# lrmantovani10/Stable-Diffusion.mojo

Measured on AMD Instinct MI355X. Metric: UNet denoising steps/sec @ 512x512 latent, batch=8, higher is better.
Workload: dtype f16; 1 GPU; Tiny-SD UNet 512x512 (latent 4x64x64), batch 8/GPU, 50-step DDPM schedule, 77-token context, no CFG, random-init weights (BASELINE configs[1]); global_batch=8, parallelism=dp1 (independent prompts, weights broadcast once)

## Files before the change

include/tsd.h:

```cpp
#ifndef TSD_H
#define TSD_H

#include <stddef.h>
#include <stdint.h>

#ifdef __cplusplus
extern "C" {
#endif

#define TSD_VERSION 100

typedef enum tsd_status {
  TSD_OK = 0,
  TSD_E_ARG = -1,
  TSD_E_SHAPE = -2,
  TSD_E_ALLOC = -3,
  TSD_E_HIP = -4,
  TSD_E_RCCL = -5,
  TSD_E_STATE = -6,
  TSD_E_NONFINITE = -7
} tsd_status;

typedef struct tsd_ctx tsd_ctx;
typedef struct tsd_model tsd_model;
// ... 310 lines not shown
enum tsd_elem_mode {
  TSD_EM_SMALL_LINEAR = 0, TSD_EM_TIME_EMBEDDING, TSD_EM_GEGLU_ERF, TSD_EM_QUICK_GELU, TSD_EM_UNARY, TSD_EM_CLIP_EMBED,
  TSD_EM_CHW_TO_NHWC, TSD_EM_IM2COL3X3, TSD_EM_NHWC_TO_CHW, TSD_EM_F32_TO_F16_ROWS, TSD_EM_F16_TO_F32_ROWS, TSD_EM_TRANSPOSE_TO_F16,
  TSD_EM_PACK_CONV, TSD_EM_PACK_LINEAR, TSD_EM_PACK_BIAS, TSD_EM_PACK_IM2COL_W, TSD_EM_ENCODER_SAMPLE, TSD_EM_COUNT
};
enum tsd_elem_operand { TSD_EO_X = 0, TSD_EO_W, TSD_EO_BIAS, TSD_EO_Y, TSD_EO_COUNT };
enum tsd_elem_info { TSD_EI_CHANGED = 0, TSD_EI_NONFINITE, TSD_EI_NB, TSD_EI_PASSES, TSD_EI_COUNT };
int tsd_debug_elem_run(tsd_ctx* ctx, const int64_t* desc, int n, const void* const* host_in, void* const* host_out, int64_t* ext,
                       int64_t* info);
int tsd_debug_gn_path_counts(tsd_ctx* ctx, int64_t* counts, int n, int reset);
int tsd_debug_jitter_selftest(tsd_ctx* ctx, int n);
int tsd_debug_model_fold(tsd_model* m, int block, void* wf, float* bf);
int tsd_debug_model_dup_fold(tsd_model* m, void* conv1_w, void* skip_w);
int64_t tsd_debug_dup_fold_host(const void* w, int rows, int taps, int ldw, int half, void* out, int ldo);
int64_t tsd_debug_ups_fold_host(const void* w, int O, int Ipad, int ldw, void* out);
int tsd_debug_model_ups_fold(tsd_model* m, int block, void* out);
int tsd_debug_set_ups_fold(tsd_ctx* ctx, int on);
int tsd_debug_model_packed_param(tsd_model* m, int index, void* out, size_t cap);
int tsd_debug_attn_bench(tsd_ctx* ctx, int B, int H, int d, int Sq, int Sk, int iters, float* ms);
int tsd_debug_attn_exact_passes(tsd_ctx* ctx, int reset);
int tsd_debug_set_attn_qb(tsd_ctx* ctx, int mode);
int tsd_debug_set_attn_diag(tsd_ctx* ctx, int on);
int tsd_debug_set_res_fuse_skip(tsd_ctx* ctx, int on);
int tsd_debug_set_qkv_fuse(tsd_ctx* ctx, int on);
int tsd_debug_set_session_hoist(tsd_ctx* ctx, int on);
int tsd_debug_set_control_stats(tsd_ctx* ctx, int on);
int tsd_debug_session_hoist_info(tsd_session* s, int64_t* info);
int tsd_debug_mfma_sustained(tsd_ctx* ctx, float ms_target, float* tflops, float* clock_ghz);

double tsd_flop_count(int kind, int L, int T);

#ifdef __cplusplus
}
#endif
#endif
```

stable-diffusion.mojo_amd/csrc/common.h:

```cpp
#pragma once
#include <hip/hip_runtime.h>
#include <stdint.h>
#include <stdio.h>
#include <string>
#include <vector>

#include "../../include/tsd.h"
#include "counter_rng.h"

typedef _Float16 half_t;

void tsd_set_error(const char* fmt, ...);
#define TSD_FAIL(code, ...)      \
  do {                           \
    tsd_set_error(__VA_ARGS__);  \
    return (code);               \
  } while (0)
#define HIP_TRY(expr)                                                                              \
  do {                                                                                             \
    hipError_t e__ = (expr);                                                                       \
    if (e__ != hipSuccess) TSD_FAIL(TSD_E_HIP, "%s failed: %s (%s:%d)", #expr, hipGetErrorString(e__), __FILE__, __LINE__); \
  } while (0)
#define TSD_TRY(expr)            \
  do {                           \
// ... 3 lines not shown

struct Arena {
  char* base = nullptr;
  size_t cap = 0, top = 0, peak = 0;
  bool planning = false;
  size_t mark() const { return top; }
  void release(size_t m) { top = m; }
  void* alloc(size_t bytes) {
    size_t a = (top + 255) & ~size_t(255);
    size_t n = a + bytes;
    if (n > peak) peak = n;
    if (!planning && n > cap) return nullptr;
    top = n;
    return planning ? (void*)(uintptr_t)(0x1000 + a) : (void*)(base + a);
  }
};

struct TsdOptions {
  int qkv_fuse = 1;
  int res_fuse_skip = 1;
  int gn_composite = 1;
  int conv_in_im2col = 1;
  int chain = 1;
  int fold_out = 1;
  int ups_fold = 1;
  int fold_dup = 1;
  int control_stats = 1;
  int session_hoist = 1;
  int conv_w_tm_mib = 2, lin_w_tm = 1, lin_w_tm_kib = 1024;
  int attn_qb = 2;
  int attn_qb_force = 0;
  int attn_wg8 = 1;
  int attn8_var = 0;
  int attn_diag = 1;
  int attn_xcd = 0;
  int xcdn = 0, conv_halo = 0, splitk = 1, splitk_mink = 4096, splitk_tiles = 256, splitk_small = 8, splitk_wide = 1, splitk_ring4 = 0,
      splitk_big = 0, sk_cfg = 5, thin_cfg = 0, tune = 15, sk256 = 0, skip128 = 1;
  int force_cfg = -1;
  int sk_big_graph = 0;
  char cfg_override[512] = "";
  int gn_apply_mult = 2;
  int gn_finalize_min = 2048;
  int debug_occ = 0;
  int debug_poison_what = 7;
  int debug_poison = -1;
  int bench_wrot = 1, bench_epi = 0, bench_altcfg = -1, gemm_ts = 0;
// ... 386 lines not shown
  const half_t* Vt = nullptr; int ldvt = 0; int64_t sVt = 0;
  half_t* O = nullptr; int ldo = 0; int64_t sO = 0;
  const float* s = nullptr;
  int B = 0, H = 0, d = 0, S = 0, N = 0;
  float scale = 1.f;
};
int launch_ip_attn_add(tsd_ctx* ctx, const IpAttnArgs& a);

struct AttnTailArgs {
  const half_t* ao = nullptr; int ld_ao = 0;
  const half_t* tok = nullptr; int ld_tok = 0;
  const half_t* x = nullptr; int ld_x = 0;
  half_t* out = nullptr; int ld_out = 0;
  const half_t* wstream = nullptr;
  const float *bso = nullptr, *bco = nullptr, *b1 = nullptr, *b2 = nullptr, *bout = nullptr;
  const half_t* Kc = nullptr; int ldk = 0; int64_t sK = 0;
  const half_t* Vt = nullptr; int ldvt = 0; int64_t sVt = 0;
  int C = 0, d = 0, heads = 0, T = 0, S = 0; int64_t M = 0;
  float scale = 1.f, eps = 1e-5f;
  float* gn_part = nullptr; int gn_nslab = 0;
};
bool attn_tail_supported(const tsd_ctx* ctx, int C, int d, int heads, int T, int64_t M, int S);
int launch_attn_tail(tsd_ctx* ctx, const AttnTailArgs& a);
size_t attn_tail_stream_bytes();
struct AttnHeadArgs {
  const half_t* x = nullptr; int ld_x = 0;
  const float* gn_stats = nullptr;
  const half_t* wstream = nullptr;
  const float* b_in = nullptr;
  half_t* tok = nullptr; int ld_tok = 0;
  half_t* qk = nullptr; int ld_qk = 0;
  half_t* vt = nullptr; int ld_vt = 0; int64_t s_vt = 0;
  int64_t M = 0; int S = 0; float eps = 1e-5f;
};
size_t attn_head_stream_bytes();
int launch_attn_head_pack(tsd_ctx* ctx, const half_t* Wc, int ld_c, const half_t* Win, int ld_in, half_t* dst);
int launch_attn_head(tsd_ctx* ctx, const AttnHeadArgs& a);
int launch_gn_stats(tsd_ctx* ctx, const half_t* x, int ld, int B, int HW, int C, int groups, float eps, float gamma, float* stats);
int launch_gn_finalize(tsd_ctx* ctx, const float* partial, int nslab, int B, int HW, int C, int groups, float eps, float gamma,
                       float* stats);
int launch_attn_tail_pack(tsd_ctx* ctx, const half_t* Wso, int ld_so, const half_t* Wq, int ld_q, const half_t* Wco, int ld_co,
                          const half_t* W1, int ld_1, const half_t* W2, int ld_2, const half_t* Wout, int ld_out, half_t* dst);
int launch_flash_attention(tsd_ctx* ctx, const AttnArgs& a);

enum { CV_SIDE = 224, CV_PATCH = 14, CV_GRID = 16, CV_PATCHES = 256, CV_PATCH_K = 588, CV_PATCH_LD = 592 };
int vision_tab(tsd_ctx* ctx, int H, int W, VisionTab* out);
// ... 3 lines not shown
```

stable-diffusion.mojo_amd/csrc/kernels_chain.hip:

```cpp
#include <math.h>
#include <stdlib.h>

#include <atomic>
#include <type_traits>

#include "common.h"
#include "lds_dma.h"

#ifndef TSD_CHAIN_ABL
#define TSD_CHAIN_ABL 0
#endif
#ifndef TSD_CHAIN_TILE_BARRIER
#define TSD_CHAIN_TILE_BARRIER 0
#endif
#ifndef TSD_CHAIN_ARES
#define TSD_CHAIN_ARES 0
#endif

typedef _Float16 h8 __attribute__((ext_vector_type(8)));
typedef _Float16 h4 __attribute__((ext_vector_type(4)));
typedef _Float16 h2 __attribute__((ext_vector_type(2)));
typedef float f4 __attribute__((ext_vector_type(4)));
typedef float f2 __attribute__((ext_vector_type(2)));

// ... 865 lines not shown
int launch_attn_tail_pack(tsd_ctx* ctx, const half_t* Wso, int ld_so, const half_t* Wq, int ld_q, const half_t* Wco, int ld_co,
                          const half_t* W1, int ld_1, const half_t* W2, int ld_2, const half_t* Wout, int ld_out, half_t* dst) {
  if (ld_so < 320 || ld_q < 320 || ld_co < 320 || ld_1 < 320 || ld_2 < 1280 || ld_out < 320)
    TSD_FAIL(TSD_E_SHAPE, "attention tail: unexpected weight pitches");
  if (!ctx->launch()) return TSD_OK;
  const int n = STREAM_BYTES / 16;
  hipLaunchKernelGGL(k_attn_tail_pack, dim3(ceil_div(n, 256)), dim3(256), 0, ctx->stream, PackSrc{Wso, ld_so}, PackSrc{Wq, ld_q},
                     PackSrc{Wco, ld_co}, PackSrc{W1, ld_1}, PackSrc{W2, ld_2}, PackSrc{Wout, ld_out}, dst);
  HIP_TRY(hipGetLastError());
  return TSD_OK;
}

int launch_attn_tail(tsd_ctx* ctx, const AttnTailArgs& a) {
  if (!attn_tail_supported(ctx, a.C, a.d, a.heads, a.T, a.M, a.S)) TSD_FAIL(TSD_E_SHAPE, "attention tail: unsupported shape");
  if (!a.wstream) TSD_FAIL(TSD_E_ARG, "attention tail: weights were not packed");
  if (a.ld_ao % 8 || a.ld_tok % 8 || a.ld_x % 8 || a.ld_out % 8 || a.ldk % 8 || a.ldvt % 8 || a.ld_ao < 320 || a.ld_tok < 320 ||
      a.ld_x < 320 || a.ld_out < 320 || a.ldk < 320 || a.ldvt < ((a.T + 7) & ~7))
    TSD_FAIL(TSD_E_SHAPE, "attention tail: misaligned or too narrow pitches");
  if ((long long)a.M * a.ld_ao * 2 >= 0x7ffffff0LL) TSD_FAIL(TSD_E_SHAPE, "attention tail: ao operand exceeds the 2 GiB addressing window");
  if (!a.ao || !a.tok || !a.x || !a.out || !a.Kc || !a.Vt || !a.bso || !a.bco || !a.b1 || !a.b2 || !a.bout)
    TSD_FAIL(TSD_E_ARG, "attention tail: NULL operand");
  if (!ctx->launch()) return TSD_OK;
  ProfScope prof(ctx, KC_CHAIN, (int)a.M, a.C, 0, 1);
  TailK k;
  k.ao = a.ao; k.tok = a.tok; k.x = a.x; k.out = a.out;
  k.ld_ao = a.ld_ao; k.ld_tok = a.ld_tok; k.ld_x = a.ld_x; k.ld_out = a.ld_out;
  k.wstream = a.wstream;
  k.bso = a.bso; k.bco = a.bco; k.b1 = a.b1; k.b2 = a.b2; k.bout = a.bout;
  k.Kc = a.Kc; k.ldk = a.ldk; k.sK = a.sK; k.Vt = a.Vt; k.ldvt = a.ldvt; k.sVt = a.sVt;
  k.T = a.T; k.M = (int)a.M; k.S = a.S;
  k.qscale = a.scale * 1.4426950408889634f; k.eps = a.eps;
  k.gn_part = a.gn_part; k.gn_nslab = a.gn_nslab;
  k.gn_stats = nullptr; k.b_in = nullptr; k.tok_out = nullptr; k.qk = nullptr; k.ld_qk = 0; k.vt = nullptr; k.ld_vt = 0; k.s_vt = 0;
  static std::atomic<unsigned long long> attr{0};
  if (!((attr.load(std::memory_order_relaxed) >> (ctx->device & 63)) & 1)) {
    HIP_TRY(hipFuncSetAttribute((const void*)attn_chain_kernel<KIND_TAIL>, hipFuncAttributeMaxDynamicSharedMemorySize, LDS_BYTES));
    attr.fetch_or(1ull << (ctx->device & 63), std::memory_order_relaxed);
  }
  hipLaunchKernelGGL(attn_chain_kernel<KIND_TAIL>, dim3((unsigned)(a.M / BM)), dim3(256), LDS_BYTES, ctx->stream, k);
  HIP_TRY(hipGetLastError());
  return TSD_OK;
}

size_t attn_head_stream_bytes() { return (size_t)HEAD_STREAM_BYTES; }

int launch_attn_head_pack(tsd_ctx* ctx, const half_t* Wc, int ld_c, const half_t* Win, int ld_in, half_t* dst) {
// ... 31 lines not shown
```

stable-diffusion.mojo_amd/csrc/runtime.cpp:

```cpp
#include <stdarg.h>
#include <stdlib.h>
#include <string.h>

#include "common.h"

static thread_local char g_err[512] = "";

void tsd_set_error(const char* fmt, ...) {
  va_list ap;
  va_start(ap, fmt);
  vsnprintf(g_err, sizeof(g_err), fmt, ap);
  va_end(ap);
}

static int env_int(const char* name, int dflt) { const char* e = getenv(name); return e && *e ? atoi(e) : dflt; }
void options_from_env(TsdOptions& o) {
  o.qkv_fuse = env_int("TSD_QKV_FUSE", o.qkv_fuse);
  o.res_fuse_skip = env_int("TSD_RES_FUSE_SKIP", o.res_fuse_skip);
  o.gn_composite = env_int("TSD_GN_COMPOSITE", o.gn_composite);
  o.conv_in_im2col = env_int("TSD_CONV_IN_IM2COL", o.conv_in_im2col);
  o.chain = env_int("TSD_CHAIN", o.chain) ? 1 : 0;
  o.fold_out = env_int("TSD_FOLD_OUT", o.fold_out) ? 1 : 0;
  o.ups_fold = env_int("TSD_UPS_FOLD", o.ups_fold) ? 1 : 0;
  o.fold_dup = env_int("TSD_FOLD_DUP", o.fold_dup) ? 1 : 0;
  o.session_hoist = env_int("TSD_SESSION_HOIST", o.session_hoist) ? 1 : 0;
  o.control_stats = env_int("TSD_CONTROL_STATS", o.control_stats) ? 1 : 0;
  o.conv_w_tm_mib = env_int("TSD_CONV_W_TM", o.conv_w_tm_mib);
  o.lin_w_tm = env_int("TSD_LIN_W_TM", o.lin_w_tm);
  o.lin_w_tm_kib = env_int("TSD_LIN_W_TM_KIB", o.lin_w_tm_kib);
  { const int q = env_int("TSD_ATTN_QB", o.attn_qb); if (q == 1 || q == 2) o.attn_qb = q; }
  o.attn_xcd = env_int("TSD_ATTN_XCD", o.attn_xcd);
  o.attn_wg8 = env_int("TSD_ATTN_WG8", o.attn_wg8) ? 1 : 0;
  o.attn8_var = env_int("TSD_ATTN8_VAR", o.attn8_var);
  o.xcdn = env_int("TSD_GEMM_XCDN", o.xcdn);
  o.conv_halo = env_int("TSD_CONV_HALO", o.conv_halo);
  o.splitk = env_int("TSD_GEMM_SPLITK", o.splitk);
  o.splitk_mink = env_int("TSD_GEMM_SPLITK_MINK", o.splitk_mink);
  o.splitk_tiles = env_int("TSD_GEMM_SPLITK_TILES", o.splitk_tiles);
  o.splitk_small = env_int("TSD_GEMM_SPLITK_SMALL", o.splitk_small);
  o.splitk_wide = env_int("TSD_GEMM_SPLITK_WIDE", o.splitk_wide);
  o.splitk_ring4 = env_int("TSD_GEMM_SPLITK_RING4", o.splitk_ring4);
// ... 193 lines not shown
```

stable-diffusion.mojo_amd/tsd/_lib.py:

```python
import ctypes as C
import os

import numpy as np

_HERE = os.path.dirname(os.path.abspath(__file__))
LIB_PATH = os.environ.get("TSD_LIB") or os.path.join(os.path.dirname(_HERE), "lib", "libtsd.so")

TSD_OK, TSD_E_ARG, TSD_E_SHAPE, TSD_E_ALLOC, TSD_E_HIP, TSD_E_RCCL, TSD_E_STATE, TSD_E_NONFINITE = 0, -1, -2, -3, -4, -5, -6, -7
os.environ.setdefault("HIP_FORCE_DEV_KERNARG", "1")

MODEL_DIFFUSION, MODEL_DECODER, MODEL_ENCODER, MODEL_CLIP, MODEL_DIFFUSION_SD15, MODEL_DIFFUSION_SD15_TORCH = 1, 2, 3, 4, 5, 6
MODEL_CLIP_TORCH, MODEL_DECODER_TORCH, MODEL_ENCODER_TORCH = 7, 8, 9
MODEL_CONTROLNET_SD15, MODEL_CONTROLNET_SD15_TORCH = 10, 11
MODEL_DIFFUSION_SD2, MODEL_CLIP_SD2 = 16, 17
MODEL_IP_ADAPTER_SD15 = 20
MODEL_CLIP_VISION_H = 22
MODEL_IP_ADAPTER_PLUS_SD15 = 24
SAMPLER_KINDS = {"ddpm": 0, "ddim": 1, "dpmpp_2m": 2}
TIMESTEP_SPACINGS = {"leading": 0, "trailing": 1}
MASK_MODES = {"area": 0, "any": 1}
PREDICTION_TYPES = {"epsilon": 0, "v": 1}


def sampler_kind(kind):
# ... 142 lines not shown
        "tsd_session_set_inpaint_seeded": ([vp, fp, fp], i),
        "tsd_session_timestep": ([vp, i], i),
        "tsd_session_upload": ([vp, fp, fp, fp, fp, f], i), "tsd_session_step": ([vp, i], i),
        "tsd_session_add_noise": ([vp, i, fp], i), "tsd_session_decode": ([vp], i),
        "tsd_session_download_latents": ([vp, fp], i), "tsd_session_download_images": ([vp, i, fp], i),
        "tsd_session_slots_open": ([vp], i), "tsd_session_slot_start": ([vp, i, fp, fp, fp, i, u64, i, f], i),
        "tsd_session_advance": ([vp, C.POINTER(C.c_uint32)], i), "tsd_session_slot_state": ([vp, i, C.POINTER(i), C.POINTER(i)], i),
        "tsd_session_slot_download": ([vp, i, fp], i), "tsd_session_slots_active": ([vp], i),
        "tsd_session_slot_set_inpaint": ([vp, i, fp, fp], i), "tsd_session_slot_inpaint_active": ([vp, i], i),
        "tsd_dist_unique_id": ([vp], i), "tsd_dist_init": ([vp, i, i, vp], i),
        "tsd_dist_broadcast_weights": ([vp, i], i), "tsd_dist_finalize": ([vp], i),
        "tsd_dist_comm_count": ([vp, C.POINTER(i)], i),
        "tsd_flop_count": ([i, i, i], C.c_double),
        "tsd_debug_splitk_errors": ([vp], i),
        "tsd_debug_xcd_round_robin": ([], i),
        "tsd_debug_nonfinite_count": ([vp, i], i),
        "tsd_debug_set_fused_attention": ([vp, i], i),
        "tsd_debug_gemm_bench": ([vp, i, i, i, i, i, i, i, i, i, i, fp], i),
        "tsd_debug_attn_bench": ([vp, i, i, i, i, i, i, fp], i),
        "tsd_debug_attn_exact_passes": ([vp, i], i),
        "tsd_debug_set_attn_qb": ([vp, i], i),
        "tsd_debug_set_attn_diag": ([vp, i], i),
        "tsd_debug_set_res_fuse_skip": ([vp, i], i),
        "tsd_debug_set_qkv_fuse": ([vp, i], i),
        "tsd_debug_set_session_hoist": ([vp, i], i),
        "tsd_debug_session_hoist_info": ([vp, C.POINTER(i64)], i),
        "tsd_debug_session_latents": ([vp, fp], i),
        "tsd_debug_mfma_sustained": ([vp, C.c_float, fp, fp], i),
        "tsd_debug_gemm_check": ([vp, i, i, i, i, i, i, i, i, i, i, fp, fp], i),
        "tsd_debug_gemm_record": ([vp, i], i),
        "tsd_debug_gemm_recorded": ([vp, i, C.POINTER(i64), i], i),
        "tsd_debug_model_fold": ([vp, i, vp, fp], i),
        "tsd_debug_model_dup_fold": ([vp, vp, vp], i),
        "tsd_debug_dup_fold_host": ([vp, i, i, i, i, vp, i], i64),
        "tsd_debug_ups_fold_host": ([vp, i, i, i, vp], i64),
        "tsd_debug_model_ups_fold": ([vp, i, vp], i),
        "tsd_debug_set_ups_fold": ([vp, i], i),
        "tsd_debug_gemm_run": ([vp, C.POINTER(i64), i, i, C.POINTER(vp), C.POINTER(vp), C.POINTER(i64), C.POINTER(i64)], i),
        "tsd_debug_gemm_plan": ([vp, C.POINTER(i64), i, i, C.POINTER(i64)], i),
        "tsd_debug_norm_run": ([vp, C.POINTER(i64), i, C.POINTER(vp), C.POINTER(vp), C.POINTER(i64), C.POINTER(i64)], i),
        "tsd_debug_attn_run": ([vp, C.POINTER(i64), i, C.POINTER(vp), C.POINTER(vp), C.POINTER(i64), C.POINTER(i64)], i),
        "tsd_debug_chain_run": ([vp, C.POINTER(i64), i, C.POINTER(vp), C.POINTER(vp), C.POINTER(i64), C.POINTER(i64)], i),
        "tsd_debug_elem_run": ([vp, C.POINTER(i64), i, C.POINTER(vp), C.POINTER(vp), C.POINTER(i64), C.POINTER(i64)], i),
        "tsd_debug_gn_path_counts": ([vp, C.POINTER(i64), i, i], i),
        "tsd_debug_jitter_selftest": ([vp, i], i),
    }
# ... 116 lines not shown
```

Before: 223.6 steps/s.

## Add 8-wave attention-tail chain kernel with a 5-slot weight ring, default on

```diff
diff --git a/include/tsd.h b/include/tsd.h
--- a/include/tsd.h
+++ b/include/tsd.h
@@ -356,6 +356,7 @@
 int tsd_debug_set_attn_qb(tsd_ctx* ctx, int mode);
 int tsd_debug_set_attn_diag(tsd_ctx* ctx, int on);
 int tsd_debug_set_res_fuse_skip(tsd_ctx* ctx, int on);
+int tsd_debug_set_chain8(tsd_ctx* ctx, int on);
 int tsd_debug_set_qkv_fuse(tsd_ctx* ctx, int on);
 int tsd_debug_set_session_hoist(tsd_ctx* ctx, int on);
 int tsd_debug_set_control_stats(tsd_ctx* ctx, int on);
diff --git a/stable-diffusion.mojo_amd/csrc/common.h b/stable-diffusion.mojo_amd/csrc/common.h
--- a/stable-diffusion.mojo_amd/csrc/common.h
+++ b/stable-diffusion.mojo_amd/csrc/common.h
@@ -49,6 +49,7 @@
   int gn_composite = 1;
   int conv_in_im2col = 1;
   int chain = 1;
+  int chain8 = 1;
   int fold_out = 1;
   int ups_fold = 1;
   int fold_dup = 1;
@@ -481,6 +482,7 @@
 };
 bool attn_tail_supported(const tsd_ctx* ctx, int C, int d, int heads, int T, int64_t M, int S);
 int launch_attn_tail(tsd_ctx* ctx, const AttnTailArgs& a);
+int launch_attn_tail8(tsd_ctx* ctx, const AttnTailArgs& a);
 size_t attn_tail_stream_bytes();
 struct AttnHeadArgs {
   const half_t* x = nullptr; int ld_x = 0;
diff --git a/stable-diffusion.mojo_amd/csrc/kernels_chain.hip b/stable-diffusion.mojo_amd/csrc/kernels_chain.hip
--- a/stable-diffusion.mojo_amd/csrc/kernels_chain.hip
+++ b/stable-diffusion.mojo_amd/csrc/kernels_chain.hip
@@ -911,6 +911,7 @@
     TSD_FAIL(TSD_E_ARG, "attention tail: NULL operand");
   if (!ctx->launch()) return TSD_OK;
   ProfScope prof(ctx, KC_CHAIN, (int)a.M, a.C, 0, 1);
+  if (ctx->opt.chain8) return launch_attn_tail8(ctx, a);
   TailK k;
   k.ao = a.ao; k.tok = a.tok; k.x = a.x; k.out = a.out;
   k.ld_ao = a.ld_ao; k.ld_tok = a.ld_tok; k.ld_x = a.ld_x; k.ld_out = a.ld_out;
diff --git a/stable-diffusion.mojo_amd/csrc/kernels_chain8.hip b/stable-diffusion.mojo_amd/csrc/kernels_chain8.hip
--- /dev/null
+++ b/stable-diffusion.mojo_amd/csrc/kernels_chain8.hip
@@ -0,0 +1,672 @@
+#include <math.h>
+#include <stdlib.h>
+
+#include <atomic>
+#include <type_traits>
+
+#include "common.h"
+#include "lds_dma.h"
+
+typedef _Float16 h8 __attribute__((ext_vector_type(8)));
+typedef _Float16 h4 __attribute__((ext_vector_type(4)));
+typedef _Float16 h2 __attribute__((ext_vector_type(2)));
+typedef float f4 __attribute__((ext_vector_type(4)));
+typedef float f2 __attribute__((ext_vector_type(2)));
+
+struct Tail8K {
+  const half_t* ao; const half_t* tok; const half_t* x; half_t* out;
+  int ld_ao, ld_tok, ld_x, ld_out;
+  const half_t* wstream;
+  const float *bso, *bco, *b1, *b2, *bout;
+  const half_t* Kc; int ldk; long long sK;
+  const half_t* Vt; int ldvt; long long sVt;
+  int T, M, S;
+  float qscale, eps;
+  float* gn_part; int gn_nslab;
+};
+
+namespace {
+constexpr int C = 320, BM = 64, FM = 2;
+constexpr int A_OFF = 0, A_KT = 8192;
+constexpr int ACT_OFF = 40960;
+constexpr int RING_OFF = ACT_OFF + 16384, SLOT = 20480, NSLOT = 5;
+constexpr int SCR_OFF = RING_OFF + NSLOT * SLOT;
+constexpr int SINK_OFF = SCR_OFF + 2048;
+constexpr int LDS_BYTES = SINK_OFF + 1024;
+static_assert(LDS_BYTES <= 163840, "LDS budget");
+constexpr int TILE_FULL = 20480, TILE_G1 = 16384;
+constexpr int SEG0_TILES = 20;
+constexpr int SEG0_BYTES = SEG0_TILES * TILE_FULL;
+constexpr int FFN_CHUNK_BYTES = 10 * TILE_G1 + 4 * TILE_FULL;
+constexpr int SEG1_TILES = 10 + 10 * 14 + 10;
+constexpr int SEG1_BYTES = 10 * TILE_FULL + 10 * FFN_CHUNK_BYTES + 10 * TILE_FULL;
+constexpr int STREAM_BYTES = SEG0_BYTES + SEG1_BYTES;
+constexpr int PPT_FULL = 3, PPT_G1 = 2;
+
+__device__ __forceinline__ float gelu_tanh_c(float x) {
+  const float k0 = -2.f * 0.7978845608028654f * 1.4426950408889634f, k1 = k0 * 0.044715f;
+  const float x2 = x * x;
+  const float t = __builtin_amdgcn_exp2f(x * __builtin_fmaf(x2, k1, k0));
+  return x * __builtin_amdgcn_rcpf(1.f + t);
+}
+template <int DMA>
+__device__ __forceinline__ void wait_vm() { wait_vm_counted<DMA, 0, PPT_FULL, PPT_G1>(); }
+__device__ __forceinline__ unsigned pin_here(unsigned w) { asm volatile("" : "+v"(w)); return w; }
+__device__ __forceinline__ void rows_swap16(float& a, float& b) { asm volatile("s_nop 1\n\tv_permlane16_swap_b32 %0, %1" : "+v"(a), "+v"(b)); }
+__device__ __forceinline__ void rows_swap32(float& a, float& b) { asm volatile("s_nop 1\n\tv_permlane32_swap_b32 %0, %1" : "+v"(a), "+v"(b)); }
+__device__ __forceinline__ float rows_sum(float v) {
+  float a = v, b = v;
+  rows_swap16(a, b);
+  a += b; b = a;
+  rows_swap32(a, b);
+  return a + b;
+}
+__device__ __forceinline__ float rows_max(float v) {
+  float a = v, b = v;
+  rows_swap16(a, b);
+  a = fmaxf(a, b); b = a;
+  rows_swap32(a, b);
+  return fmaxf(a, b);
+}
+__device__ __forceinline__ void lds_barrier() {
+  tsd_jitter();
+  asm volatile("s_waitcnt lgkmcnt(0)" ::: "memory");
+  __builtin_amdgcn_s_barrier();
+  asm volatile("" ::: "memory");
+}
+__device__ __forceinline__ int wswz(int rho) { return 3 * ((rho >> 2) & 1); }
+}
+
+__global__ __launch_bounds__(512, 1) void attn_tail8_kernel(const Tail8K p) {
+  extern __shared__ __attribute__((aligned(16))) char smem[];
+  const int tid = threadIdx.x, lane = tid & 63;
+  const int wave = __builtin_amdgcn_readfirstlane(tid >> 6);
+  const int wn = wave & 3, wm = wave >> 2;
+  const int r0 = wm * 32;
+  const int rsel = lane & 15, key = lane & 7, g = lane >> 4;
+  const int lrow = lane >> 3, cch = (lane & 7) ^ lrow;
+  const int m0 = blockIdx.x * BM;
+  const int bsmp = m0 / p.S;
+
+  auto tile_off = [&](int seg, int gi, bool& g1, bool& live) {
+    g1 = false; live = true;
+    if (seg == 0) { live = gi < SEG0_TILES; return gi * TILE_FULL; }
+    if (gi < 10) return SEG0_BYTES + gi * TILE_FULL;
+    if (gi < 150) {
+      const int q = gi - 10;
+      int jc, r; bool second;
+      if (q < 10) { jc = 0; r = q; second = false; }
+      else if (q < 136) { const int pq = (q - 10) / 14, pr = (q - 10) - 14 * pq; second = pr >= 10; jc = second ? pq : pq + 1; r = second ? pr - 10 : pr; }
+      else { jc = 9; r = q - 136; second = true; }
+      const int base = SEG0_BYTES + 10 * TILE_FULL + jc * FFN_CHUNK_BYTES;
+      if (!second) { g1 = true; return base + r * TILE_G1; }
+      return base + 10 * TILE_G1 + r * TILE_FULL;
+    }
+    live = gi < SEG1_TILES;
+    return SEG0_BYTES + 10 * TILE_FULL + 10 * FFN_CHUNK_BYTES + (gi - 150) * TILE_FULL;
+  };
+  const rsrc_t rw = make_rsrc(p.wstream, STREAM_BYTES), rdead = make_rsrc(p.wstream, 0);
+  const unsigned lane16 = lane * 16;
+  auto piece = [&](int off, bool g1, bool live, int slot, int i) {
+    const int pi = wm * (g1 ? PPT_G1 : PPT_FULL) + i;
+    const bool real = pi < (g1 ? 4 : 5);
+    const int j = wn * (g1 ? 4 : 5) + pi;
+    blds16(live && real ? rw : rdead, lane16, (unsigned)(off + j * 1024),
+           real ? smem + RING_OFF + slot * SLOT + wn * 5120 + pi * 1024 : smem + SINK_OFF);
+  };
+  int gt = 0, sl = 0;
+  auto seg_begin = [&](int seg) {
+    gt = 0; sl = 0;
+#pragma unroll
+    for (int t = 0; t < 4; t++) {
+      bool g1, live;
+      const int off = tile_off(seg, t, g1, live);
+#pragma unroll
+      for (int i = 0; i < PPT_FULL; i++) if (!(g1 && i >= PPT_G1)) piece(off, g1, live, t, i);
+    }
+  };
+
+  const int a_rd = (r0 + rsel) * 128;
+  const int w_rd = rsel * 64 + ((g ^ wswz(rsel)) << 4);
+  auto gemm = [&](auto seg_c, f4 (&acc)[FM][5], int a_base, int nk) {
+    constexpr int FN = 5, SEG = decltype(seg_c)::value;
+#pragma unroll
+    for (int a = 0; a < FM; a++)
+#pragma unroll
+      for (int b = 0; b < FN; b++) acc[a][b] = f4{0.f, 0.f, 0.f, 0.f};
+    h8 afA[FM], wfA[FN], afB[FM], wfB[FN];
+    auto step = [&](int kt, h8 (&af)[FM], h8 (&wf)[FN], const h8 (&paf)[FM], const h8 (&pwf)[FN], bool have_prev, bool have_next) {
+      bool g1 = false, live = false;
+      int off = 0, s4 = 0;
+      const char *sA = smem, *sW = smem;
+      if (have_next) {
+        tsd_jitter();
+        int younger = 0;
+#pragma unroll
+        for (int d = 1; d <= 3; d++) { bool yg1, ylive; tile_off(SEG, gt + d, yg1, ylive); younger += yg1 ? PPT_G1 : PPT_FULL; }
+        wait_alt_begin();
+        switch (younger) {
+          case 6: wait_vm<6>(); break;
+          case 7: wait_vm<7>(); break;
+          case 8: wait_vm<8>(); break;
+          default: wait_vm<9>(); break;
+        }
+        wait_alt_end();
+        asm volatile("s_waitcnt lgkmcnt(0)" ::: "memory");
+        __builtin_amdgcn_s_barrier();
+        asm volatile("" ::: "memory");
+        sA = smem + a_base + (kt >> 1) * A_KT + a_rd + ((((kt & 1) * 4 + g) ^ key) << 4);
+        sW = smem + RING_OFF + sl * SLOT + wn * 5120 + w_rd;
+        off = tile_off(SEG, gt + 4, g1, live);
+        s4 = sl == 0 ? 4 : sl - 1;
+      }
+      constexpr int NM = FM * FN, NR = FM + FN;
+      if (!have_prev) {
+#pragma unroll
+        for (int a = 0; a < FM; a++) af[a] = *(const h8*)(sA + a * 2048);
+#pragma unroll
+        for (int b = 0; b < FN; b++) wf[b] = *(const h8*)(sW + b * 1024);
+#pragma unroll
+        for (int i = 0; i < PPT_FULL; i++) if (!(g1 && i >= PPT_G1)) piece(off, g1, live, s4, i);
+      } else {
+#pragma unroll
+        for (int q = 0; q < NM; q++) {
+          const int b = q >> 1, a = q & 1;
+          acc[a][b] = __builtin_amdgcn_mfma_f32_16x16x32_f16(pwf[b], paf[a], acc[a][b], 0, 0, 0);
+          if (have_next) {
+            __builtin_amdgcn_sched_barrier(0);
+            if (q < NR) {
+              if (q < FM) af[q] = *(const h8*)(sA + q * 2048);
+              else wf[q - FM] = *(const h8*)(sW + (q - FM) * 1024);
+            }
+            if (q == 2 || q == 5 || q == 8) {
+              const int i = q / 3;
+              if (!(g1 && i >= PPT_G1)) piece(off, g1, live, s4, i);
+            }
+            __builtin_amdgcn_sched_barrier(0);
+          }
+        }
+      }
+      if (have_next) {
+        gt++;
+        sl = sl == 4 ? 0 : sl + 1;
+      }
+    };
+    for (int kt = 0; kt < nk; kt += 2) {
+      step(kt, afA, wfA, afB, wfB, kt > 0, true);
+      step(kt + 1, afB, wfB, afA, wfA, true, true);
+    }
+    step(nk, afA, wfA, afB, wfB, true, false);
+  };
+  using I0 = std::integral_constant<int, 0>;
+  using I1 = std::integral_constant<int, 1>;
+
+  const int cbase = wn * 80 + g * 20;
+  auto load_cols = [&](const float* vec, f4 (&bv)[5]) {
+#pragma unroll
+    for (int b = 0; b < 5; b++) bv[b] = *(const f4*)(vec + cbase + b * 4);
+  };
+  auto load_rows_raw = [&](const half_t* src, int ld, h4 (&raw)[FM][5]) {
+#pragma unroll
+    for (int a = 0; a < FM; a++) {
+      const half_t* rp = src + (long long)(m0 + r0 + a * 16 + rsel) * ld + cbase;
+#pragma unroll
+      for (int b = 0; b < 5; b++) raw[a][b] = *(const h4*)(rp + b * 4);
+    }
+  };
+  auto a_piece = [&](int row, int col) { return (col >> 6) * A_KT + row * 128 + ((((col >> 3) & 7) ^ (row & 7)) << 4) + (col & 4) * 2; };
+  int apo[5];
+#pragma unroll
+  for (int b = 0; b < 5; b++) apo[b] = A_OFF + a_piece(r0 + rsel, cbase + b * 4);
+  auto store_a_tile = [&](const f4 (&v)[FM][5], const float (&mul)[FM], const float (&sub)[FM]) {
+#pragma unroll
+    for (int a = 0; a < FM; a++) {
+#pragma unroll
+      for (int b = 0; b < 5; b++) {
+        h4 o;
+#pragma unroll
+        for (int r = 0; r < 4; r++) o[r] = (half_t)((v[a][b][r] - sub[a]) * mul[a]);
+        *(h4*)(smem + apo[b] + a * 2048) = o;
+      }
+    }
+  };
+  float* scr = (float*)(smem + SCR_OFF);
+  auto layernorm_to_a = [&](const f4 (&v)[FM][5]) {
+    float mw[FM], m2w[FM];
+#pragma unroll
+    for (int a = 0; a < FM; a++) {
+      float t = 0.f;
+#pragma unroll
+      for (int b = 0; b < 5; b++) t += (v[a][b][0] + v[a][b][1]) + (v[a][b][2] + v[a][b][3]);
+      t = rows_sum(t);
+      mw[a] = t * (1.f / 80.f);
+      float u = 0.f;
+#pragma unroll
+      for (int b = 0; b < 5; b++)
+#pragma unroll
+        for (int r = 0; r < 4; r++) { const float d = v[a][b][r] - mw[a]; u += d * d; }
+      u = rows_sum(u);
+      m2w[a] = u;
+      if (g == 0) *(f2*)(scr + ((r0 + a * 16 + rsel) * 4 + wn) * 2) = f2{mw[a], u};
+    }
+    lds_barrier();
+    float mean[FM], rs[FM];
+#pragma unroll
+    for (int a = 0; a < FM; a++) {
+      const f4 p01 = *(const f4*)(scr + (r0 + a * 16 + rsel) * 8), p23 = *(const f4*)(scr + (r0 + a * 16 + rsel) * 8 + 4);
+      const float mu = 0.25f * ((p01[0] + p01[2]) + (p23[0] + p23[2]));
+      const float d0 = p01[0] - mu, d1 = p01[2] - mu, d2 = p23[0] - mu, d3 = p23[2] - mu;
+      const float m2 = ((p01[1] + p01[3]) + (p23[1] + p23[3])) + 80.f * ((d0 * d0 + d1 * d1) + (d2 * d2 + d3 * d3));
+      mean[a] = mu;
+      rs[a] = 1.f / (sqrtf(m2 * (1.f / C)) + p.eps);
+    }
+    store_a_tile(v, rs, mean);
+  };
+  const float oneM[FM] = {1.f, 1.f}, zeroM[FM] = {0.f, 0.f};
+
+  f4 T[FM][5];
+  f4 acc[FM][5];
+  f4 bv[5];
+  h4 raw[FM][5];
+  {
+    const rsrc_t ra = make_rsrc(p.ao);
+#pragma unroll
+    for (int i = 0; i < 5; i++) {
+      const int j = wave + 8 * i, kt = j >> 3, row = (j & 7) * 8 + lrow;
+      blds16(ra, (unsigned)((m0 + row) * p.ld_ao + cch * 8) * 2, kt * 128, smem + A_OFF + kt * A_KT + (j & 7) * 1024);
+    }
+  }
+  seg_begin(0);
+  load_rows_raw(p.tok, p.ld_tok, raw);
+  load_cols(p.bso, bv);
+  gemm(I0{}, acc, A_OFF, 10);
+#pragma unroll
+  for (int a = 0; a < FM; a++)
+#pragma unroll
+    for (int b = 0; b < 5; b++)
+#pragma unroll
+      for (int r = 0; r < 4; r++) T[a][b][r] = (float)raw[a][b][r] + (acc[a][b][r] + bv[b][r]);
+  layernorm_to_a(T);
+  gemm(I0{}, acc, A_OFF, 10);
+  wait_vm<0>();
+  lds_barrier();
+  constexpr int KT_B = 80 * 128, V0_OFF = 5 * KT_B, V1_OFF = V0_OFF + 320 * 128;
+  static_assert(V1_OFF + 320 * 32 <= NSLOT * SLOT, "context tiles must fit in the ring region");
+  {
+    const rsrc_t rk = make_rsrc(p.Kc + bsmp * p.sK), rv = make_rsrc(p.Vt + bsmp * p.sVt);
+    const int nch = (p.T + 7) >> 3;
+#pragma unroll
+    for (int m = 0; m < 2; m++) {
+      const int rb = wave + 8 * m;
+      if (rb < 10) {
+        const int rho = rb * 8 + lrow, b = rho >> 4, ii = rho & 15;
+        const int kidx = b < 4 ? 32 * (b >> 1) + 8 * (ii >> 2) + 4 * (b & 1) + (ii & 3) : 64 + ii;
+        const unsigned live = (unsigned)((kidx - p.T) >> 31);
+        const unsigned koff = (((unsigned)(kidx * p.ldk + cch * 8) * 2) & live) | (PAD_OFF & ~live);
+#pragma unroll
+        for (int kt = 0; kt < 5; kt++) blds16(rk, koff, kt * 128, smem + RING_OFF + kt * KT_B + rb * 1024);
+      }
+    }
+    const unsigned vlive0 = (unsigned)((cch - nch) >> 31), vlive1 = (unsigned)((8 + (lane & 1) - nch) >> 31);
+    const unsigned v0off = (((unsigned)(lrow * p.ldvt + cch * 8) * 2) & vlive0) | (PAD_OFF & ~vlive0);
+    const unsigned v1off = (((unsigned)((lane >> 1) * p.ldvt + (8 + (lane & 1)) * 8) * 2) & vlive1) | (PAD_OFF & ~vlive1);
+#pragma unroll
+    for (int i = 0; i < 5; i++) {
+      const int q = wave + 8 * i;
+      blds16(rv, v0off, (unsigned)(q * 8 * p.ldvt) * 2, smem + RING_OFF + V0_OFF + q * 1024);
+    }
+#pragma unroll
+    for (int i = 0; i < 2; i++) {
+      const int q = wave + 8 * i;
+      if (q < 10) blds16(rv, v1off, (unsigned)(q * 32 * p.ldvt) * 2, smem + RING_OFF + V1_OFF + q * 1024);
+    }
+  }
+  {
+    const float qsM[FM] = {p.qscale, p.qscale};
+    store_a_tile(acc, qsM, zeroM);
+  }
+  load_cols(p.bco, bv);
+  wait_vm<0>();
+  lds_barrier();
+  const bool t_ge64 = p.T >= 64;
+  f4 mk4;
+#pragma unroll
+  for (int r = 0; r < 4; r++) mk4[r] = 64 + 4 * g + r >= p.T ? -1.0e30f : 0.f;
+#pragma unroll
+  for (int hh = 0; hh < 2; hh++) {
+    const int h = wn * 2 + hh, c0 = h * 5;
+    f4 sc[FM][5];
+#pragma unroll
+    for (int a = 0; a < FM; a++)
+#pragma unroll
+      for (int b = 0; b < 5; b++) sc[a][b] = f4{0.f, 0.f, 0.f, 0.f};
+#pragma unroll
+    for (int st = 0; st < 2; st++) {
+      const int cg = st == 0 ? c0 + g : c0 + 4;
+      const int ktile = cg >> 3, cpos = cg & 7;
+      h8 qa[FM], kb[5];
+#pragma unroll
+      for (int a = 0; a < FM; a++) qa[a] = *(const h8*)(smem + A_OFF + ktile * A_KT + a_rd + a * 2048 + ((cpos ^ key) << 4));
+#pragma unroll
+      for (int b = 0; b < 5; b++) {
+        kb[b] = *(const h8*)(smem + RING_OFF + ktile * KT_B + (b * 16 + rsel) * 128 + ((cpos ^ key) << 4));
+        if (st == 1 && g != 0) kb[b] = h8{0, 0, 0, 0, 0, 0, 0, 0};
+      }
+#pragma unroll
+      for (int a = 0; a < FM; a++)
+#pragma unroll
+        for (int b = 0; b < 5; b++) sc[a][b] = __builtin_amdgcn_mfma_f32_16x16x32_f16(kb[b], qa[a], sc[a][b], 0, 0, 0);
+    }
+    h8 pf[FM][3];
+#pragma unroll
+    for (int a = 0; a < FM; a++) {
+      if (!t_ge64) {
+#pragma unroll
+        for (int b = 0; b < 4; b++)
+#pragma unroll
+          for (int r = 0; r < 4; r++)
+            if (32 * (b >> 1) + 8 * g + 4 * (b & 1) + r >= p.T) sc[a][b][r] = -1.0e30f;
+      }
+      sc[a][4] += mk4;
+      float mx = sc[a][0][0];
+#pragma unroll
+      for (int b = 0; b < 5; b++)
+#pragma unroll
+        for (int r = 0; r < 4; r++) mx = fmaxf(mx, sc[a][b][r]);
+      mx = rows_max(mx);
+#pragma unroll
+      for (int kk = 0; kk < 3; kk++) {
+        h8 o = h8{0, 0, 0, 0, 0, 0, 0, 0};
+#pragma unroll
+        for (int j = 0; j < (kk < 2 ? 8 : 4); j++) o[j] = (half_t)__builtin_amdgcn_exp2f(sc[a][kk < 2 ? 2 * kk + (j >> 2) : 4][j & 3] - mx);
+        pf[a][kk] = o;
+      }
+    }
+    f4 oc[FM][3];
+#pragma unroll
+    for (int a = 0; a < FM; a++)
+#pragma unroll
+      for (int b = 0; b < 3; b++) oc[a][b] = f4{0.f, 0.f, 0.f, 0.f};
+#pragma unroll
+    for (int kk = 0; kk < 3; kk++) {
+      h8 vb[3];
+#pragma unroll
+      for (int b = 0; b < 3; b++) {
+        const int row = min(h * 40 + b * 16 + rsel, C - 1);
+        if (kk < 2) vb[b] = *(const h8*)(smem + RING_OFF + V0_OFF + row * 128 + (((kk * 4 + g) ^ (row & 7)) << 4));
+        else {
+          const h4 lo = *(const h4*)(smem + RING_OFF + V1_OFF + row * 32 + g * 8);
+          vb[b] = h8{lo[0], lo[1], lo[2], lo[3], 0, 0, 0, 0};
+        }
+      }
+      if (rsel == 8) vb[2] = kk < 2 ? h8{1, 1, 1, 1, 1, 1, 1, 1} : h8{1, 1, 1, 1, 0, 0, 0, 0};
+#pragma unroll
+      for (int a = 0; a < FM; a++)
+#pragma unroll
+        for (int b = 0; b < 3; b++) oc[a][b] = __builtin_amdgcn_mfma_f32_16x16x32_f16(vb[b], pf[a][kk], oc[a][b], 0, 0, 0);
+    }
+    float rinv[FM];
+#pragma unroll
+    for (int a = 0; a < FM; a++) rinv[a] = 1.f / rows_sum(g == 2 ? oc[a][2][0] : 0.f);
+#pragma unroll
+    for (int a = 0; a < FM; a++) {
+      const int row = r0 + a * 16 + rsel;
+#pragma unroll
+      for (int b = 0; b < 3; b++) {
+        const int d = b * 16 + 4 * g;
+        if (d < 40) {
+          h4 o;
+#pragma unroll
+          for (int r = 0; r < 4; r++) o[r] = (half_t)(oc[a][b][r] * rinv[a]);
+          *(h4*)(smem + A_OFF + a_piece(row, h * 40 + d)) = o;
+        }
+      }
+    }
+  }
+  lds_barrier();
+  seg_begin(1);
+  gemm(I1{}, acc, A_OFF, 10);
+#pragma unroll
+  for (int a = 0; a < FM; a++)
+#pragma unroll
+    for (int b = 0; b < 5; b++) T[a][b] += acc[a][b] + bv[b];
+  layernorm_to_a(T);
+  f4 acc2[FM][5];
+#pragma unroll
+  for (int a = 0; a < FM; a++)
+#pragma unroll
+    for (int b = 0; b < 5; b++) acc2[a][b] = f4{0.f, 0.f, 0.f, 0.f};
+  {
+    f4 b1v[4];
+    unsigned oreg[FM][4];
+    h8 afS[2][FM], wfS[2][5];
+    auto load_b1 = [&](int jc) {
+      const float* bp = p.b1 + jc * 256 + wn * 64 + g * 16;
+#pragma unroll
+      for (int b = 0; b < 4; b++) b1v[b] = *(const f4*)(bp + b * 4);
+    };
+    auto act_pair = [&](int u, int jp) {
+      const f4 v = acc[u][jp];
+      const float o0 = v[0] * gelu_tanh_c(v[1]), o1 = v[2] * gelu_tanh_c(v[3]);
+      h2 pk = {(half_t)o0, (half_t)o1};
+      oreg[u][jp] = pin_here(__builtin_bit_cast(unsigned, pk));
+    };
+    auto write_act = [&]() {
+      typedef unsigned u4v __attribute__((ext_vector_type(4)));
+#pragma unroll
+      for (int a = 0; a < FM; a++)
+        *(u4v*)(smem + ACT_OFF + (wn >> 1) * A_KT + (r0 + a * 16 + rsel) * 128 + ((((wn & 1) * 4 + g) ^ key) << 4)) =
+            u4v{oreg[a][0], oreg[a][1], oreg[a][2], oreg[a][3]};
+    };
+    constexpr int F_BIAS = 1, F_WRITE = 4, F_PLAIN = 8;
+    constexpr int FB = SEG0_BYTES + 10 * TILE_FULL;
+    int jb = FB;
+    auto gstep = [&](auto pk_c, auto ck_c, auto kc_c, auto set_c, auto fill_c, auto flags_c, auto lk_c, auto loff_c, auto yg_c) {
+      constexpr int PK = decltype(pk_c)::value, CK = decltype(ck_c)::value, KC = decltype(kc_c)::value, SET = decltype(set_c)::value;
+      constexpr int FILL = decltype(fill_c)::value, FLAGS = decltype(flags_c)::value;
+      constexpr int LK = decltype(lk_c)::value, LOFF = decltype(loff_c)::value, YG = decltype(yg_c)::value;
+      constexpr int FNp = PK == 1 ? 4 : 5, FNc = CK == 1 ? 4 : 5;
+      constexpr bool G1N = LK == 1;
+      int s4 = 0;
+      const char *sA = smem, *sW = smem;
+      if constexpr (CK != 0) {
+        tsd_jitter();
+        wait_vm<YG>();
+        asm volatile("s_waitcnt lgkmcnt(0)" ::: "memory");
+        __builtin_amdgcn_s_barrier();
+        asm volatile("" ::: "memory");
+        sA = smem + (CK == 1 ? A_OFF : ACT_OFF) + (KC >> 1) * A_KT + a_rd + ((((KC & 1) * 4 + g) ^ key) << 4);
+        sW = smem + RING_OFF + sl * SLOT + wn * 5120 + w_rd;
+        s4 = sl == 0 ? 4 : sl - 1;
+      }
+      const int off = jb + LOFF;
+      auto dma = [&](int i) {
+        if constexpr (CK != 0 && LK != 0) { if (!(G1N && i >= PPT_G1)) piece(off, G1N, true, s4, i); }
+      };
+      if constexpr ((FLAGS & F_WRITE) != 0) write_act();
+      h8 (&af)[FM] = afS[SET];
+      h8 (&wf)[5] = wfS[SET];
+      const h8 (&paf)[FM] = afS[SET ^ 1];
+      const h8 (&pwf)[5] = wfS[SET ^ 1];
+      if constexpr (PK == 0) {
+        if constexpr (CK != 0) {
+#pragma unroll
+          for (int a = 0; a < FM; a++) af[a] = *(const h8*)(sA + a * 2048);
+#pragma unroll
+          for (int b = 0; b < FNc; b++) wf[b] = *(const h8*)(sW + b * 1024);
+#pragma unroll
+          for (int i = 0; i < PPT_FULL; i++) dma(i);
+        }
+      } else {
+        constexpr int NM = FM * FNp, NR = CK != 0 ? FM + FNc : 0;
+        static_assert(NR <= NM, "a fragment read behind every MFMA at the most");
+#pragma unroll
+        for (int q = 0; q < NM; q++) {
+          const int b = q >> 1, a = q & 1;
+          if constexpr (PK == 1) {
+            const f4 c0 = (FLAGS & F_BIAS) ? b1v[b] : acc[a][b];
+            acc[a][b] = __builtin_amdgcn_mfma_f32_16x16x32_f16(pwf[b], paf[a], c0, 0, 0, 0);
+          } else {
+            acc2[a][b] = __builtin_amdgcn_mfma_f32_16x16x32_f16(pwf[b], paf[a], acc2[a][b], 0, 0, 0);
+          }
+          __builtin_amdgcn_sched_barrier(0);
+          if (q < NR) {
+            if (q < FM) af[q] = *(const h8*)(sA + q * 2048);
+            else wf[q - FM] = *(const h8*)(sW + (q - FM) * 1024);
+          }
+          if (q == (NM == 10 ? 2 : 1)) dma(0);
+          if (q == (NM == 10 ? 5 : 4)) dma(1);
+          if (q == NM - 1) dma(2);
+          if (FILL >= 0 && NM == 10 && q % 5 == 4) { const int ip = FILL * 2 + q / 5; act_pair(ip >> 2, ip & 3); }
+          __builtin_amdgcn_sched_barrier(0);
+        }
+      }
+      if constexpr ((FLAGS & F_PLAIN) != 0) {
+#pragma unroll
+        for (int u = 0; u < FM; u++)
+#pragma unroll
+          for (int jp = 0; jp < 4; jp++) act_pair(u, jp);
+        write_act();
+      }
+      if constexpr (CK != 0) {
+        gt++;
+        sl = sl == 4 ? 0 : sl + 1;
+      }
+    };
+#define TSD_IC(x) std::integral_constant<int, (x)>{}
+    auto la_kind = [](int pd, bool last) constexpr { return pd < 10 ? 1 : (pd < 14 ? 2 : (last ? 2 : 1)); };
+    auto la_off = [](int pd, bool last) constexpr {
+      return pd < 10 ? pd * TILE_G1
+                     : (pd < 14 ? -FFN_CHUNK_BYTES + 10 * TILE_G1 + (pd - 10) * TILE_FULL
+                                : (last ? 10 * TILE_G1 + (pd - 14) * TILE_FULL : FFN_CHUNK_BYTES + (pd - 14) * TILE_G1));
+    };
+    auto la_yg = [=](int p_, bool last) constexpr {
+      int y = 0;
+      for (int d = 1; d <= 3; d++) y += la_kind(p_ + d, last) == 1 ? PPT_G1 : PPT_FULL;
+      return y;
+    };
+    auto iteration = [&](auto first_c, auto last_c) {
+      constexpr bool FIRST = decltype(first_c)::value, LAST = decltype(last_c)::value;
+#define TSD_LA(P) TSD_IC(la_kind((P) + 4, LAST)), TSD_IC(la_off((P) + 4, LAST)), TSD_IC(la_yg((P), LAST))
+      if constexpr (FIRST) gstep(TSD_IC(1), TSD_IC(1), TSD_IC(0), TSD_IC(0), TSD_IC(-1), TSD_IC(F_PLAIN), TSD_LA(0));
+      else gstep(TSD_IC(2), TSD_IC(1), TSD_IC(0), TSD_IC(0), TSD_IC(3), TSD_IC(0), TSD_LA(0));
+      gstep(TSD_IC(1), TSD_IC(1), TSD_IC(1), TSD_IC(1), TSD_IC(-1), TSD_IC(FIRST ? F_BIAS : F_BIAS | F_WRITE), TSD_LA(1));
+      gstep(TSD_IC(1), TSD_IC(1), TSD_IC(2), TSD_IC(0), TSD_IC(-1), TSD_IC(0), TSD_LA(2));
+      gstep(TSD_IC(1), TSD_IC(1), TSD_IC(3), TSD_IC(1), TSD_IC(-1), TSD_IC(0), TSD_LA(3));
+      gstep(TSD_IC(1), TSD_IC(1), TSD_IC(4), TSD_IC(0), TSD_IC(-1), TSD_IC(0), TSD_LA(4));
+      if constexpr (!LAST) load_b1((jb - FB) / FFN_CHUNK_BYTES + 1);
+      gstep(TSD_IC(1), TSD_IC(1), TSD_IC(5), TSD_IC(1), TSD_IC(-1), TSD_IC(0), TSD_LA(5));
+      gstep(TSD_IC(1), TSD_IC(1), TSD_IC(6), TSD_IC(0), TSD_IC(-1), TSD_IC(0), TSD_LA(6));
+      gstep(TSD_IC(1), TSD_IC(1), TSD_IC(7), TSD_IC(1), TSD_IC(-1), TSD_IC(0), TSD_LA(7));
+      gstep(TSD_IC(1), TSD_IC(1), TSD_IC(8), TSD_IC(0), TSD_IC(-1), TSD_IC(0), TSD_LA(8));
+      gstep(TSD_IC(1), TSD_IC(1), TSD_IC(9), TSD_IC(1), TSD_IC(-1), TSD_IC(0), TSD_LA(9));
+      gstep(TSD_IC(1), TSD_IC(2), TSD_IC(0), TSD_IC(0), TSD_IC(-1), TSD_IC(0), TSD_LA(10));
+      gstep(TSD_IC(2), TSD_IC(2), TSD_IC(1), TSD_IC(1), TSD_IC(0), TSD_IC(0), TSD_LA(11));
+      gstep(TSD_IC(2), TSD_IC(2), TSD_IC(2), TSD_IC(0), TSD_IC(1), TSD_IC(0), TSD_LA(12));
+      gstep(TSD_IC(2), TSD_IC(2), TSD_IC(3), TSD_IC(1), TSD_IC(2), TSD_IC(0), TSD_LA(13));
+#undef TSD_LA
+    };
+    load_b1(0);
+#define TSD_LA0(P) TSD_IC(1), TSD_IC((P) + 4 < 10 ? ((P) + 4) * TILE_G1 : FFN_CHUNK_BYTES + ((P) + 4 - 10) * TILE_G1), TSD_IC(3 * PPT_G1)
+    gstep(TSD_IC(0), TSD_IC(1), TSD_IC(0), TSD_IC(0), TSD_IC(-1), TSD_IC(0), TSD_LA0(0));
+    gstep(TSD_IC(1), TSD_IC(1), TSD_IC(1), TSD_IC(1), TSD_IC(-1), TSD_IC(F_BIAS), TSD_LA0(1));
+    gstep(TSD_IC(1), TSD_IC(1), TSD_IC(2), TSD_IC(0), TSD_IC(-1), TSD_IC(0), TSD_LA0(2));
+    gstep(TSD_IC(1), TSD_IC(1), TSD_IC(3), TSD_IC(1), TSD_IC(-1), TSD_IC(0), TSD_LA0(3));
+    gstep(TSD_IC(1), TSD_IC(1), TSD_IC(4), TSD_IC(0), TSD_IC(-1), TSD_IC(0), TSD_LA0(4));
+    load_b1(1);
+    gstep(TSD_IC(1), TSD_IC(1), TSD_IC(5), TSD_IC(1), TSD_IC(-1), TSD_IC(0), TSD_LA0(5));
+    gstep(TSD_IC(1), TSD_IC(1), TSD_IC(6), TSD_IC(0), TSD_IC(-1), TSD_IC(0), TSD_LA0(6));
+    gstep(TSD_IC(1), TSD_IC(1), TSD_IC(7), TSD_IC(1), TSD_IC(-1), TSD_IC(0), TSD_LA0(7));
+    gstep(TSD_IC(1), TSD_IC(1), TSD_IC(8), TSD_IC(0), TSD_IC(-1), TSD_IC(0), TSD_LA0(8));
+    gstep(TSD_IC(1), TSD_IC(1), TSD_IC(9), TSD_IC(1), TSD_IC(-1), TSD_IC(0), TSD_LA0(9));
+#undef TSD_LA0
+    jb = FB + FFN_CHUNK_BYTES;
+    iteration(std::true_type{}, std::false_type{});
+    for (int j = 2; j < 9; j++) {
+      jb += FFN_CHUNK_BYTES;
+      iteration(std::false_type{}, std::false_type{});
+    }
+    jb += FFN_CHUNK_BYTES;
+    iteration(std::false_type{}, std::true_type{});
+    gstep(TSD_IC(2), TSD_IC(0), TSD_IC(0), TSD_IC(0), TSD_IC(3), TSD_IC(0), TSD_IC(0), TSD_IC(0), TSD_IC(0));
+    lds_barrier();
+    write_act();
+    gstep(TSD_IC(0), TSD_IC(2), TSD_IC(0), TSD_IC(0), TSD_IC(-1), TSD_IC(0), TSD_IC(2), TSD_IC(FFN_CHUNK_BYTES + 0 * TILE_FULL), TSD_IC(3 * PPT_FULL));
+    gstep(TSD_IC(2), TSD_IC(2), TSD_IC(1), TSD_IC(1), TSD_IC(-1), TSD_IC(0), TSD_IC(2), TSD_IC(FFN_CHUNK_BYTES + 1 * TILE_FULL), TSD_IC(3 * PPT_FULL));
+    gstep(TSD_IC(2), TSD_IC(2), TSD_IC(2), TSD_IC(0), TSD_IC(-1), TSD_IC(0), TSD_IC(2), TSD_IC(FFN_CHUNK_BYTES + 2 * TILE_FULL), TSD_IC(3 * PPT_FULL));
+    gstep(TSD_IC(2), TSD_IC(2), TSD_IC(3), TSD_IC(1), TSD_IC(-1), TSD_IC(0), TSD_IC(2), TSD_IC(FFN_CHUNK_BYTES + 3 * TILE_FULL), TSD_IC(3 * PPT_FULL));
+    gstep(TSD_IC(2), TSD_IC(0), TSD_IC(0), TSD_IC(0), TSD_IC(-1), TSD_IC(0), TSD_IC(0), TSD_IC(0), TSD_IC(0));
+#undef TSD_IC
+  }
+  load_cols(p.b2, bv);
+#pragma unroll
+  for (int a = 0; a < FM; a++)
+#pragma unroll
+    for (int b = 0; b < 5; b++) T[a][b] += acc2[a][b] + bv[b];
+  store_a_tile(T, oneM, zeroM);
+  load_cols(p.bout, bv);
+  load_rows_raw(p.x, p.ld_x, raw);
+  gemm(I1{}, acc, A_OFF, 10);
+  float gs1[2] = {0.f, 0.f}, gs2[2] = {0.f, 0.f};
+  lds_barrier();
+  constexpr int RP = 656;
+  static_assert(A_OFF + 64 * RP <= RING_OFF, "output staging must stay clear of the ring (dead DMAs may still land there)");
+#pragma unroll
+  for (int a = 0; a < FM; a++) {
+#pragma unroll
+    for (int b = 0; b < 5; b++) {
+      h4 o;
+#pragma unroll
+      for (int r = 0; r < 4; r++) {
+        o[r] = (half_t)((float)raw[a][b][r] + (acc[a][b][r] + bv[b][r]));
+        const float f = (float)o[r];
+        const int grp = (b * 4 + r) / 10;
+        gs1[grp] += f; gs2[grp] += f * f;
+      }
+      *(h4*)(smem + A_OFF + (r0 + a * 16 + rsel) * RP + (cbase + b * 4) * 2) = o;
+    }
+  }
+  lds_barrier();
+#pragma unroll
+  for (int i = 0; i < 5; i++) {
+    const int t = tid + 512 * i, row = t / 40, c = t - row * 40;
+    *(h8*)(p.out + (long long)(m0 + row) * p.ld_out + c * 8) = *(const h8*)(smem + A_OFF + row * RP + c * 16);
+  }
+  if (p.gn_part) {
+#pragma unroll
+    for (int k = 0; k < 2; k++) {
+#pragma unroll
+      for (int o = 1; o < 16; o <<= 1) { gs1[k] += __shfl_xor(gs1[k], o); gs2[k] += __shfl_xor(gs2[k], o); }
+    }
+    if (rsel == 0) {
+      const int mrow = m0 + r0, bb = mrow / p.S, slab = (mrow - bb * p.S) >> 5;
+      float* ob = p.gn_part + (((long long)bb * p.gn_nslab + slab) * 32 + wn * 8 + g * 2) * 2;
+      *(f4*)ob = f4{gs1[0], gs2[0], gs1[1], gs2[1]};
+    }
+  }
+  wait_vm<0>();
+}
+
+extern "C" int tsd_debug_set_chain8(tsd_ctx* ctx, int on) {
+  return ctx_set_option(ctx, &TsdOptions::chain8, on ? 1 : 0, 0, 1);
+}
+
+int launch_attn_tail8(tsd_ctx* ctx, const AttnTailArgs& a) {
+  Tail8K k;
+  k.ao = a.ao; k.tok = a.tok; k.x = a.x; k.out = a.out;
+  k.ld_ao = a.ld_ao; k.ld_tok = a.ld_tok; k.ld_x = a.ld_x; k.ld_out = a.ld_out;
+  k.wstream = a.wstream;
+  k.bso = a.bso; k.bco = a.bco; k.b1 = a.b1; k.b2 = a.b2; k.bout = a.bout;
+  k.Kc = a.Kc; k.ldk = a.ldk; k.sK = a.sK; k.Vt = a.Vt; k.ldvt = a.ldvt; k.sVt = a.sVt;
+  k.T = a.T; k.M = (int)a.M; k.S = a.S;
+  k.qscale = a.scale * 1.4426950408889634f; k.eps = a.eps;
+  k.gn_part = a.gn_part; k.gn_nslab = a.gn_nslab;
+  static std::atomic<unsigned long long> attr{0};
+  if (!((attr.load(std::memory_order_relaxed) >> (ctx->device & 63)) & 1)) {
+    HIP_TRY(hipFuncSetAttribute((const void*)attn_tail8_kernel, hipFuncAttributeMaxDynamicSharedMemorySize, LDS_BYTES));
+    attr.fetch_or(1ull << (ctx->device & 63), std::memory_order_relaxed);
+  }
+  hipLaunchKernelGGL(attn_tail8_kernel, dim3((unsigned)(a.M / BM)), dim3(512), LDS_BYTES, ctx->stream, k);
+  HIP_TRY(hipGetLastError());
+  return TSD_OK;
+}
diff --git a/stable-diffusion.mojo_amd/csrc/runtime.cpp b/stable-diffusion.mojo_amd/csrc/runtime.cpp
--- a/stable-diffusion.mojo_amd/csrc/runtime.cpp
+++ b/stable-diffusion.mojo_amd/csrc/runtime.cpp
@@ -17,6 +17,7 @@
 void options_from_env(TsdOptions& o) {
   o.qkv_fuse = env_int("TSD_QKV_FUSE", o.qkv_fuse);
   o.res_fuse_skip = env_int("TSD_RES_FUSE_SKIP", o.res_fuse_skip);
+  o.chain8 = env_int("TSD_CHAIN8", o.chain8);
   o.gn_composite = env_int("TSD_GN_COMPOSITE", o.gn_composite);
   o.conv_in_im2col = env_int("TSD_CONV_IN_IM2COL", o.conv_in_im2col);
   o.chain = env_int("TSD_CHAIN", o.chain) ? 1 : 0;
diff --git a/stable-diffusion.mojo_amd/tsd/_lib.py b/stable-diffusion.mojo_amd/tsd/_lib.py
--- a/stable-diffusion.mojo_amd/tsd/_lib.py
+++ b/stable-diffusion.mojo_amd/tsd/_lib.py
@@ -188,6 +188,7 @@
         "tsd_debug_set_attn_qb": ([vp, i], i),
         "tsd_debug_set_attn_diag": ([vp, i], i),
         "tsd_debug_set_res_fuse_skip": ([vp, i], i),
+        "tsd_debug_set_chain8": ([vp, i], i),
         "tsd_debug_set_qkv_fuse": ([vp, i], i),
         "tsd_debug_set_session_hoist": ([vp, i], i),
         "tsd_debug_session_hoist_info": ([vp, C.POINTER(i64)], i),
```

Result: no change. 224.1 steps/s (median of 6 runs) (+0.2%).
